# bacpop/ska.rust

Hardware: AMD Instinct MI355X
Metric: genomes/sec ska build+align, 1 000x5 Mbp k=31; bit-exact vs CPU (higher is better)
Workload: dtype u64

## Files before the change

ska.rust_amd/csrc/skx_device.hip:

```cpp
#include "skx_device.h"
#include <cstdlib>

namespace skx {

HashParams make_hash_params(int k)
{
    HashParams p;
    p.bits = 2 * (k - 1);
    p.hb = k - 1;
    p.hmask = p.hb >= 32 ? ~0u : ((1u << p.hb) - 1);
    p.c[0] = 0x9E3779B1u; p.c[1] = 0x85EBCA6Bu; p.c[2] = 0xC2B2AE35u; p.c[3] = 0x27D4EB2Fu;
    return p;
}

__device__ static inline uint32_t revcomp_arm(uint32_t x, int n)
{
    x = __builtin_bitreverse32(x);
    x = ((x >> 1) & 0x55555555u) | ((x & 0x55555555u) << 1);
    x ^= 0xAAAAAAAAu;
    return n ? x >> (32 - 2 * n) : 0;
}

__device__ static inline void pack16(const uint32_t w[4], uint32_t &code, uint32_t &bad, uint32_t &nl)
{
// ... 15 lines not shown
}
__device__ static inline void pack16_nonl(const uint32_t w[4], uint32_t &code, uint32_t &bad)
{
    code = 0; bad = 0;
    uint32_t c0f = 0x0F0F0F0Fu, c7f = 0x7F7F7F7Fu;
    asm volatile("" : "+v"(c0f), "+v"(c7f));
#pragma unroll
    for (int i = 0; i < 4; i++) {
        uint32_t x = w[i];
        uint32_t c = (x >> 1) & 0x03030303u;
        code = (code << 8) | ((c * 0x40100401u) >> 24);
        uint32_t t = (x & c0f) ^ 0x0E0E0E0Eu;
        uint32_t nzt = (t + c7f) & 0x80808080u;
        uint32_t u = x ^ 0x0A0A0A0Au;
        uint32_t znl = ~(((u & c7f) + c7f) | u | c7f);
        uint32_t fb = (((~nzt) & 0x80808080u) | znl) >> 7;
        bad |= (((fb * 0x01020408u) >> 24) & 0xFu) << (4 * i);
    }
}
__device__ static inline uint32_t qualbad16(const uint32_t w[4], int min_qual)
{
    uint32_t m = 0;
#pragma unroll
    for (int i = 0; i < 4; i++)
#pragma unroll
        for (int b = 0; b < 4; b++) {
            uint32_t q = (w[i] >> (8 * b)) & 0xFF;
            m |= (uint32_t)(((q - 33u) & 0xFFu) <= (uint32_t)min_qual) << (4 * i + b);
        }
    return m;
}

__device__ static inline uint32_t block_excl_scan(uint32_t v, uint32_t *s_tmp, uint32_t *total);
__device__ static inline uint32_t block_excl_scan_row(uint32_t v, uint32_t *s_tmp, uint32_t *total, int tid);

#ifdef SKX_PHASE_PROF
__device__ unsigned long long g_phase_prof[1024 * 16];
#define PHASE_PROF_(i) do { if (threadIdx.x == 0) { const unsigned long long t_ = __builtin_readcyclecounter(); atomicAdd(&g_phase_prof[(blockIdx.x & 1023) * 16 + (i)], t_ - tprof); tprof = t_; } } while (0)
#define PHASE_PROF_START unsigned long long tprof = __builtin_readcyclecounter()
extern "C" void skx_debug_phase_prof(unsigned long long *out, int reset)
{
    static unsigned long long h[1024 * 16];
    (void)hipDeviceSynchronize();
    (void)hipMemcpyFromSymbol(h, HIP_SYMBOL(g_phase_prof), sizeof(h));
    for (int i = 0; i < 16; i++) { out[i] = 0; for (int j = 0; j < 1024; j++) out[i] += h[j * 16 + i]; }
    if (reset) { for (auto &x : h) x = 0; (void)hipMemcpyToSymbol(HIP_SYMBOL(g_phase_prof), h, sizeof(h)); }
}
#else
#define PHASE_PROF_(i) do { } while (0)
#define PHASE_PROF_START do { } while (0)
#endif
#if defined(SKX_PHASE_PROF) && SKX_PHASE_PROF == 1
#define EXT_PROF(i) do { if (SCATTER) PHASE_PROF_(i); } while (0)
#else
#define EXT_PROF(i) do { } while (0)
#endif
#if defined(SKX_PHASE_PROF) && SKX_PHASE_PROF == 4
#define UN_PROF(i) do { if ((threadIdx.x & 63) == 0) { const unsigned long long t_ = __builtin_readcyclecounter(); atomicAdd(&g_phase_prof[(blockIdx.x & 1023) * 16 + (i)], t_ - tprof); tprof = t_; } } while (0)
#define UN_WAIT() asm volatile("s_waitcnt vmcnt(0)" ::: "memory")
#else
#define UN_PROF(i) do { } while (0)
#define UN_WAIT() do { } while (0)
#endif
#if defined(SKX_PHASE_PROF) && SKX_PHASE_PROF == 2
#define DD_PROF(i) PHASE_PROF_(i)
#else
#define DD_PROF(i) do { } while (0)
#endif
template <bool SCATTER, int TILE, bool HI, int PPT, bool SPLIT, int RMAX>
__global__ __launch_bounds__(TILE / PPT, SPLIT ? 6 : 1) void extract_kernel(ExtractArgs a)
{
    constexpr int NT = TILE / PPT;
    constexpr int NCH = PPT / 16;
    constexpr int NCHUNK = TILE / 16 + 5;
    extern __shared__ __attribute__((aligned(16))) unsigned char s_raw[];
    const int B = 1 << a.logB;
    uint32_t *s_hist = reinterpret_cast<uint32_t *>(s_raw);
    uint32_t *s_base = s_hist + B + 4;
    uint32_t *s_tmp = s_base + B;
    unsigned char *s_rest = reinterpret_cast<unsigned char *>(s_tmp + 20);
    uint32_t *s_code = reinterpret_cast<uint32_t *>(s_rest);
    uint16_t *s_bad = reinterpret_cast<uint16_t *>(s_code + NCHUNK + 3);
    uint16_t *s_qbad = s_bad + NCHUNK + 3;
    uint64_t *s_stage = reinterpret_cast<uint64_t *>(s_rest);

    const int tid = threadIdx.x;
    PHASE_PROF_START;
    const uint64_t per_group = 8ull * (uint64_t)a.tiles_max;
    const uint64_t L = blockIdx.x;
    int sample; uint64_t tile;
    if (a.parts > 1) {
        const int v = (int)(L & 7u);
        if (v >= a.n_samples * a.parts) return;
        sample = v / a.parts; tile = (uint64_t)(v % a.parts) * (uint64_t)a.tiles_part + (L >> 3);
        if (tile >= (uint64_t)a.tiles_max || (L >> 3) >= (uint64_t)a.tiles_part) return;
    } else { sample = (int)((L / per_group) * 8 + (L % per_group) % 8); tile = (L % per_group) / 8; }
    if (sample >= a.n_samples) return;
    const uint64_t len = a.lens[sample];
    const uint64_t T0 = tile * TILE;
    if (T0 >= len) return;
    typedef const uint8_t __attribute__((address_space(1))) *gbytes_t;
    typedef uint32_t u32x4 __attribute__((ext_vector_type(4)));
    typedef const u32x4 __attribute__((address_space(1))) *gvec_t;
    gbytes_t seq = (gbytes_t)(uintptr_t)a.seqs[sample];
    gbytes_t qual = a.quals ? (gbytes_t)(uintptr_t)a.quals[sample] : (gbytes_t)0;

    const int k = a.k, h = (k - 1) / 2;
    const HashParams hp = a.hp;
    const int hb = hp.hb;
    const int bshift = hp.bits - a.logB;
    const int bsh_hi = hp.bits + 4 - 32 - a.logB;
    const uint32_t rcflag = a.rc ? ~0u : 0u;
    const bool top_from_hl = a.logB <= hb;
    const int top_shift = top_from_hl ? hb - a.logB : 0;
    const uint32_t am = (1u << (2 * h)) - 1;

    for (int i = tid; i < B + 4; i += NT) s_hist[i] = 0;
    for (int c = tid; c < NCHUNK; c += NT) {
        const int64_t p = (int64_t)T0 - 64 + 16 * (int64_t)c;
        uint32_t w[4], q[4] = {0, 0, 0, 0};
        if (p >= 0 && (uint64_t)p + 16 <= len) {
            const u32x4 v = *(gvec_t)(seq + p);
            w[0] = v.x; w[1] = v.y; w[2] = v.z; w[3] = v.w;
            if (qual) { const u32x4 u = *(gvec_t)(qual + p); q[0] = u.x; q[1] = u.y; q[2] = u.z; q[3] = u.w; }
        } else {
#pragma unroll
            for (int i = 0; i < 4; i++) {
                uint32_t x = 0, y = 0;
#pragma unroll
                for (int b = 0; b < 4; b++) {
                    int64_t pos = p + 4 * i + b;
                    bool in = pos >= 0 && (uint64_t)pos < len;
                    x |= (uint32_t)(in ? seq[pos] : (uint8_t)'\n') << (8 * b);
                    if (qual) y |= (uint32_t)(in ? qual[pos] : (uint8_t)'~') << (8 * b);
                }
                w[i] = x; q[i] = y;
            }
        }
        uint32_t code, bad;
        pack16_nonl(w, code, bad);
        uint32_t qb = 0;
        if (qual) {
            uint32_t c2, b2, nl;
            pack16(w, c2, b2, nl);
            qb = qualbad16(q, a.min_qual) & ~nl;
            if (a.qual_filter == 2) bad |= qb;
        }
        s_code[c] = code; s_bad[c] = (uint16_t)bad; if (qual) s_qbad[c] = (uint16_t)qb;
    }
    __syncthreads();
    EXT_PROF(0);
    constexpr uint64_t PF_AHEAD = 20;
    uint32_t pfw = 0;
    if (SCATTER && tid < TILE / 128) {
        uint64_t pos = T0 + PF_AHEAD * TILE + (uint64_t)tid * 128;
        gbytes_t ps = seq;
        uint64_t plen = len;
        if (T0 + PF_AHEAD * TILE >= len && sample + 8 < a.n_samples) {
            pos = (tile + PF_AHEAD - (len + TILE - 1) / TILE) * TILE + (uint64_t)tid * 128;
            ps = (gbytes_t)(uintptr_t)a.seqs[sample + 8]; plen = a.lens[sample + 8];
        }
        if (pos + 4 <= plen) pfw = *(const uint32_t __attribute__((address_space(1))) *)(ps + pos);
    }

    uint64_t wv[PPT];
    uint32_t rk[PPT];
    {
    const int c0 = tid * NCH + 4;
    const uint64_t prev = ((uint64_t)s_code[c0 - 2] << 32) | s_code[c0 - 1];
    uint32_t lower = (uint32_t)prev & am;
    uint32_t mid = (uint32_t)(prev >> (2 * h)) & 3u;
    uint32_t upper = (uint32_t)(prev >> (2 * h + 2)) & am;
    uint32_t rc_upper = revcomp_arm(lower, h), rc_lower = revcomp_arm(upper, h), rc_mid = mid ^ 2u;
#pragma unroll
    for (int half = 0; half < NCH; half++) {
        const int c = c0 + half;
        const uint64_t G = ~((uint64_t)s_bad[c - 2] | ((uint64_t)s_bad[c - 1] << 16) | ((uint64_t)s_bad[c] << 32)) & 0xFFFFFFFFFFFFull;
        uint64_t Wk = ~0ull;
        {
            uint64_t A = G; int offset = 0, span = 1;
            for (int bit = 0; bit < 6; bit++) {
                if ((k >> bit) & 1) { Wk &= A << offset; offset += span; }
                A &= A << span; span <<= 1;
            }
        }
        uint64_t V = Wk;
        const uint64_t cand = Wk & ~(G << k) & ((~G >> 1) | ((uint64_t)(s_bad[c + 1] & 1u) << 47)) & (0xFFFFull << 32);
        if (cand) {
            const int64_t pc = (int64_t)T0 - 64 + 16 * (int64_t)c;
            uint32_t m = (uint32_t)(cand >> 32);
            while (m) {
                const int j = __builtin_ctz(m); m &= m - 1;
                const uint64_t pos = (uint64_t)(pc + j + 1);
                if (pos >= len || seq[pos] == (uint8_t)'\n') V &= ~(1ull << (32 + j));
            }
        }
        if (qual && a.qual_filter != 0)
            V &= ~((((uint64_t)s_qbad[c - 2] | ((uint64_t)s_qbad[c - 1] << 16) | ((uint64_t)s_qbad[c] << 32))) << h);
        const uint32_t vm = (uint32_t)(V >> 32) & 0xFFFFu;
        const uint32_t cw = s_code[c];
#pragma unroll
        for (int j = 0; j < 16; j++) {
            const uint32_t code = (cw >> (30 - 2 * j)) & 3u;
            upper = ((upper << 2) | mid) & am;
            mid = lower >> (2 * h - 2);
            lower = ((lower << 2) | code) & am;
            rc_lower = (rc_lower >> 2) | (rc_mid << (2 * h - 2));
            rc_mid = mid ^ 2u;
            rc_upper = (rc_upper >> 2) | ((code ^ 2u) << (2 * h - 2));
            const uint64_t kf = ((uint64_t)upper << 32) | lower, kr = ((uint64_t)rc_upper << 32) | rc_lower;
            const bool gt = kf > kr && rcflag;
            const bool eq = kf == kr && rcflag;
            uint32_t hl = gt ? rc_upper : upper, hr = gt ? rc_lower : lower;
            const uint32_t m4 = (1u << (gt ? rc_mid : mid)) | (eq ? (1u << rc_mid) : 0u);
            hmix_halves(hl, hr, hp);
            const uint64_t w = ((uint64_t)hl << (hb + 4)) | ((uint64_t)hr << 4) | m4;
            wv[16 * half + j] = w;
            const bool valid = (vm >> j) & 1u;
            const uint32_t bk = valid ? (top_from_hl ? hl >> top_shift : (uint32_t)((w >> 4) >> bshift)) : (uint32_t)B;
            const uint32_t r = atomicAdd(&s_hist[bk], 1u);
            rk[16 * half + j] = (bk << 16) | r;
        }
    }
    }
    __syncthreads();
    EXT_PROF(1);
    uint32_t *ghist = a.hist + ((uint64_t)sample << a.logB);
    if (!SCATTER) {
        for (int i = tid; i < B; i += NT) { uint32_t n = s_hist[i]; if (n) atomicAdd(&ghist[i], n); }
        return;
    }
    const int R = (B + NT - 1) / NT;
    const int b0 = tid * R < B ? tid * R : B, b1 = b0 + R < B ? b0 + R : B;
    uint32_t gb[RMAX], lsum = 0;
#pragma unroll
    for (int r = 0; r < RMAX; r++) {
        gb[r] = 0;
        if (b0 + r < b1) { const uint32_t n = s_hist[b0 + r]; if (n) gb[r] = atomicAdd(&ghist[b0 + r], n); lsum += n; }
    }
    uint32_t total;
    uint32_t lrun = block_excl_scan_row(lsum, s_tmp, &total, tid);
    EXT_PROF(2);
#pragma unroll
    for (int r = 0; r < RMAX; r++)
        if (b0 + r < b1) { const uint32_t n = s_hist[b0 + r]; s_hist[b0 + r] = lrun; lrun += n; }
    if (tid == 0) s_hist[B] = total;
    __syncthreads();
    EXT_PROF(3);
    constexpr uint32_t HALF = SPLIT ? TILE / 2 : TILE;
    uint32_t sidx_[SPLIT ? PPT : 1];
#pragma unroll
    for (int j = 0; j < PPT; j++) {
        const uint32_t idx = s_hist[rk[j] >> 16] + (rk[j] & 0xFFFFu);
        if (SPLIT) sidx_[j] = idx;
        if (idx < HALF) s_stage[idx] = wv[j];
    }
    const uint64_t *off = a.off + ((uint64_t)sample << a.logB);
    const bool fixed = a.capacity != 0xFFFFFFFFu;
    const uint64_t span0 = fixed ? ((uint64_t)sample << a.logB) * a.capacity : off[0];
    bool dropped = false;
#pragma unroll
    for (int r = 0; r < RMAX; r++)
        if (b0 + r < b1) {
            const uint32_t b = (uint32_t)(b0 + r), start = s_hist[b], n = s_hist[b + 1] - start;
            const bool over = n && gb[r] + n > a.capacity;
            if (over) dropped = true;
            s_base[b] = over ? 0u - start : (fixed ? b * a.capacity : (uint32_t)(off[b] - off[0])) + gb[r] - start;
        }
    asm volatile("" :: "v"(pfw));
    __syncthreads();
    EXT_PROF(4);
    typedef uint64_t __attribute__((address_space(1))) *gout_t;
    gout_t out = (gout_t)(uintptr_t)(a.words + span0);
    const uint32_t end0 = total < HALF ? total : HALF;
    for (uint32_t i = tid; i < end0; i += NT) {
        const uint64_t w = s_stage[i];
        const uint32_t b = HI ? (uint32_t)(w >> 32) >> bsh_hi : (uint32_t)((w >> 4) >> bshift);
        out[s_base[b] + i] = w;
    }
    EXT_PROF(5);
    if (SPLIT && total > HALF) {
        __syncthreads();
        EXT_PROF(6);
#pragma unroll
        for (int j = 0; j < PPT; j++) if (sidx_[j] - HALF < HALF) s_stage[sidx_[j] - HALF] = wv[j];
        __syncthreads();
        EXT_PROF(7);
        for (uint32_t i = HALF + tid; i < total; i += NT) {
            const uint64_t w = s_stage[i - HALF];
            const uint32_t b = HI ? (uint32_t)(w >> 32) >> bsh_hi : (uint32_t)((w >> 4) >> bshift);
            out[s_base[b] + i] = w;
        }
    }
    EXT_PROF(8);
    if (dropped) *a.overflow = 1;
}
template <int TILE, bool SPLIT>
static inline size_t extract_lds(const ExtractArgs &a, bool scatter)
{
    size_t codes = (size_t)(TILE / 16 + 8) * 8 + 64;
    size_t stage = scatter ? (size_t)TILE * (SPLIT ? 4 : 8) : 0;
    return ((size_t)8 << a.logB) + 16 + 80 + (stage > codes ? stage : codes);
}
static inline void extract_parts(ExtractArgs &a)
{
    a.parts = 0; a.tiles_part = 0;
    if (a.n_samples >= 1 && a.n_samples < 8 && a.tiles_max >= 64) { a.parts = 8 / a.n_samples; a.tiles_part = (a.tiles_max + a.parts - 1) / a.parts; if (a.parts < 2) a.parts = 0; }
}
template <bool SCATTER, int TILE, bool HI, int PPT, bool SPLIT, int RMAX>
static void launch_extract_t(const ExtractArgs &a_, hipStream_t st)
{
    ExtractArgs a = a_;
    extract_parts(a);
    const uint64_t g = a.parts > 1 ? 8ull * (uint64_t)a.tiles_part : (((uint64_t)a.n_samples + 7) / 8) * 8ull * (uint64_t)a.tiles_max;
    if (!g) return;
    const size_t lds = extract_lds<TILE, SPLIT>(a, SCATTER);
    (void)hipFuncSetAttribute((const void *)extract_kernel<SCATTER, TILE, HI, PPT, SPLIT, RMAX>, hipFuncAttributeMaxDynamicSharedMemorySize, (int)lds);
    hipLaunchKernelGGL((extract_kernel<SCATTER, TILE, HI, PPT, SPLIT, RMAX>), dim3((unsigned)g), dim3(TILE / PPT), lds, st, a);
}
template <bool SCATTER>
static void launch_extract(const ExtractArgs &a, hipStream_t st)
{
    const bool hi = a.hp.bits + 4 - 32 - a.logB >= 0;
    if (a.logB <= 10) {
        if (hi) launch_extract_t<SCATTER, 12288, true, 16, SCATTER, 2>(a, st); else launch_extract_t<SCATTER, 12288, false, 16, SCATTER, 2>(a, st);
    } else if (a.logB == 11) {
        if (hi) launch_extract_t<SCATTER, 12288, true, 16, SCATTER, 4>(a, st); else launch_extract_t<SCATTER, 12288, false, 16, SCATTER, 4>(a, st);
    } else {
        if (hi) launch_extract_t<SCATTER, 8192, true, 16, SCATTER, 16>(a, st); else launch_extract_t<SCATTER, 8192, false, 16, SCATTER, 16>(a, st);
    }
}
int extract_tile_bases(int logB) { return logB <= 11 ? 12288 : 8192; }
void launch_hist(const ExtractArgs &a, hipStream_t st) { launch_extract<false>(a, st); }
void launch_scatter(const ExtractArgs &a, hipStream_t st)
{
    launch_extract<true>(a, st);
}
__device__ static inline uint32_t wave_incl_scan(uint32_t v)
{
    const int lane = threadIdx.x & 63;
#pragma unroll
    for (int d = 1; d < 64; d <<= 1) { uint32_t t = __shfl_up(v, d, 64); if (lane >= d) v += t; }
    return v;
}
__device__ static inline uint32_t block_excl_scan(uint32_t v, uint32_t *s_tmp , uint32_t *total)
{
    const int lane = threadIdx.x & 63, wv = threadIdx.x >> 6, nw = (blockDim.x + 63) >> 6;
    uint32_t inc = wave_incl_scan(v);
    if (lane == 63) s_tmp[wv] = inc;
    __syncthreads();
    if (threadIdx.x == 0) { uint32_t run = 0; for (int i = 0; i < nw; i++) { uint32_t t = s_tmp[i]; s_tmp[i] = run; run += t; } s_tmp[16] = run; }
    __syncthreads();
    uint32_t r = s_tmp[wv] + inc - v;
    if (total) *total = s_tmp[16];
    __syncthreads();
    return r;
}

__device__ static inline uint32_t wave_incl_scan_dpp(uint32_t v)
{
    uint32_t inc = v;
    inc += (uint32_t)__builtin_amdgcn_update_dpp(0, (int)inc, 0x111, 0xf, 0xf, true);
    inc += (uint32_t)__builtin_amdgcn_update_dpp(0, (int)inc, 0x112, 0xf, 0xf, true);
    inc += (uint32_t)__builtin_amdgcn_update_dpp(0, (int)inc, 0x114, 0xf, 0xf, true);
    inc += (uint32_t)__builtin_amdgcn_update_dpp(0, (int)inc, 0x118, 0xf, 0xf, true);
    inc += (uint32_t)__builtin_amdgcn_update_dpp(0, (int)inc, 0x142, 0xa, 0xf, false);
    inc += (uint32_t)__builtin_amdgcn_update_dpp(0, (int)inc, 0x143, 0xc, 0xf, false);
    return inc;
}
__device__ static inline uint32_t block_excl_scan_row(uint32_t v, uint32_t *s_tmp , uint32_t *total, int tid)
{
    const int lane = tid & 63;
    const int wv = __builtin_amdgcn_readfirstlane(tid >> 6), nw = (int)((blockDim.x + 63) >> 6);
    const uint32_t inc = wave_incl_scan_dpp(v);
    if (lane == 63) s_tmp[wv] = inc;
    __syncthreads();
    uint32_t t = lane < nw ? s_tmp[lane & 15] : 0u;
    t += (uint32_t)__builtin_amdgcn_update_dpp(0, (int)t, 0x111, 0xf, 0xf, true);
    t += (uint32_t)__builtin_amdgcn_update_dpp(0, (int)t, 0x112, 0xf, 0xf, true);
    t += (uint32_t)__builtin_amdgcn_update_dpp(0, (int)t, 0x114, 0xf, 0xf, true);
    t += (uint32_t)__builtin_amdgcn_update_dpp(0, (int)t, 0x118, 0xf, 0xf, true);
    const uint32_t before = wv ? (uint32_t)__builtin_amdgcn_readlane((int)t, wv - 1) : 0u;
    if (total) *total = (uint32_t)__builtin_amdgcn_readlane((int)t, nw - 1);
    return before + inc - v;
}

__global__ __launch_bounds__(1024) void scan_u32_kernel(const uint32_t *in, uint64_t *out, uint64_t n, uint32_t *max_out)
{
    __shared__ uint32_t s_tmp[17];
    __shared__ uint32_t s_max;
    uint64_t carry = 0;
    uint32_t mx = 0;
    if (threadIdx.x == 0) s_max = 0;
    for (uint64_t base = 0; base < n; base += 4096) {
        uint32_t v[4]; uint32_t sum = 0;
#pragma unroll
        for (int i = 0; i < 4; i++) { uint64_t idx = base + (uint64_t)threadIdx.x * 4 + i; v[i] = idx < n ? in[idx] : 0; sum += v[i]; mx = v[i] > mx ? v[i] : mx; }
        uint32_t tot;
        uint32_t ex = block_excl_scan(sum, s_tmp, &tot);
        uint64_t run = carry + ex;
#pragma unroll
        for (int i = 0; i < 4; i++) { uint64_t idx = base + (uint64_t)threadIdx.x * 4 + i; if (idx < n) out[idx] = run; run += v[i]; }
        carry += tot;
    }
    if (threadIdx.x == 0) out[n] = carry;
    if (max_out) { atomicMax(&s_max, mx); __syncthreads(); if (threadIdx.x == 0) *max_out = s_max; }
}
__global__ void fill_offsets_kernel(uint64_t *off, uint64_t n, uint32_t capacity)
{
    for (uint64_t i = blockIdx.x * (uint64_t)blockDim.x + threadIdx.x; i <= n; i += (uint64_t)gridDim.x * blockDim.x) off[i] = i * capacity;
}
void launch_fill_offsets(uint64_t *off, uint64_t n, uint32_t capacity, hipStream_t st)
{
    hipLaunchKernelGGL(fill_offsets_kernel, dim3(1024), dim3(256), 0, st, off, n, capacity);
}
void launch_scan_u32(const uint32_t *in, uint64_t *out, uint64_t n, uint32_t *max_out, hipStream_t st)
{
    hipLaunchKernelGGL(scan_u32_kernel, dim3(1), dim3(1024), 0, st, in, out, n, max_out);
}

constexpr int SCAN8_PER_BLOCK = 8192;
__global__ __launch_bounds__(1024) void scan_u8_sums_kernel(const uint8_t *in, uint64_t n, uint32_t *sums)
{
    __shared__ uint32_t s_tmp[17];
    const uint64_t base = (uint64_t)blockIdx.x * SCAN8_PER_BLOCK + (uint64_t)threadIdx.x * 8;
    uint32_t sum = 0;
    if (base + 8 <= n) { uint64_t v = *reinterpret_cast<const uint64_t *>(in + base); for (int i = 0; i < 8; i++) sum += ((v >> (8 * i)) & 0xFF) == 1; }
    else for (int i = 0; i < 8; i++) sum += (base + i < n) && in[base + i] == 1;
    uint32_t tot; block_excl_scan(sum, s_tmp, &tot);
    if (threadIdx.x == 0) sums[blockIdx.x] = tot;
}
__global__ __launch_bounds__(1024) void scan_u8_apply_kernel(const uint8_t *in, uint64_t n, const uint64_t *block_off, uint64_t *out)
{
    __shared__ uint32_t s_tmp[17];
    const uint64_t base = (uint64_t)blockIdx.x * SCAN8_PER_BLOCK + (uint64_t)threadIdx.x * 8;
    uint32_t v[8]; uint32_t sum = 0;
    for (int i = 0; i < 8; i++) { v[i] = (base + i < n) && in[base + i] == 1; sum += v[i]; }
    uint32_t ex = block_excl_scan(sum, s_tmp, nullptr);
    uint64_t run = block_off[blockIdx.x] + ex;
    for (int i = 0; i < 8; i++) { if (base + i < n) out[base + i] = run; run += v[i]; }
    if (blockIdx.x == gridDim.x - 1 && threadIdx.x == blockDim.x - 1) out[n] = run;
}
uint64_t scan_u8_blocks(uint64_t n) { return (n + SCAN8_PER_BLOCK - 1) / SCAN8_PER_BLOCK; }
void launch_scan_u8(const uint8_t *flags, uint64_t *pos, uint64_t n, uint32_t *sums, uint64_t *offs, hipStream_t st)
{
    const uint64_t nb = scan_u8_blocks(n);
    if (nb == 0) { (void)hipMemsetAsync(pos, 0, 8, st); return; }
    hipLaunchKernelGGL(scan_u8_sums_kernel, dim3((unsigned)nb), dim3(1024), 0, st, flags, n, sums);
    hipLaunchKernelGGL(scan_u32_kernel, dim3(1), dim3(1024), 0, st, (const uint32_t *)sums, offs, nb, (uint32_t *)nullptr);
    hipLaunchKernelGGL(scan_u8_apply_kernel, dim3((unsigned)nb), dim3(1024), 0, st, flags, n, (const uint64_t *)offs, pos);
}

constexpr uint32_t TABLE_PAD = 128;

template <bool HI>
__device__ static inline uint32_t word_field(uint64_t w, int sh, uint32_t mask)
{
    return HI ? ((uint32_t)(w >> 32) >> (sh - 32)) & mask : (uint32_t)(w >> sh) & mask;
}

__device__ static inline uint32_t home_slot(uint64_t w, int rem_bits, uint32_t nslots)
{
    uint32_t l32;
    if (rem_bits >= 32) {
        const int sh = rem_bits - 28;
        l32 = sh >= 32 ? (uint32_t)(w >> 32) : __builtin_amdgcn_alignbit((uint32_t)(w >> 32), (uint32_t)w, (uint32_t)sh);
    } else {
        l32 = rem_bits == 0 ? 0u : (uint32_t)(((w >> 4) & ((1ull << rem_bits) - 1)) << (32 - rem_bits));
    }
    return __umulhi(l32, nslots);
}
template <bool FAST>
__device__ static inline uint32_t home_slot_t(uint64_t w, int rem_bits, uint32_t nslots)
{
    if (FAST) return __umulhi(__builtin_amdgcn_alignbit((uint32_t)(w >> 32), (uint32_t)w, (uint32_t)(rem_bits - 28)), nslots);
    return home_slot(w, rem_bits, nslots);
}
__device__ static inline bool table_insert(unsigned long long *tab, uint32_t total_slots, uint32_t home, uint64_t w)
{
    const uint64_t key = w >> 4;
    for (uint32_t i = home; i < total_slots; ++i) {
        unsigned long long old = tab[i];
        if (old == 0ull) old = atomicCAS(&tab[i], 0ull, (unsigned long long)w);
        if (old == 0ull) return true;
        if ((old >> 4) == key) {
            if ((old | w) != old) atomicOr(&tab[i], (unsigned long long)(w & 15ull));
            return true;
        }
    }
    return false;
}
__device__ static inline int table_insert_slot(unsigned long long *tab, uint32_t total_slots, uint32_t home, uint64_t w, uint32_t &slot)
{
    const uint64_t key = w >> 4;
    for (uint32_t i = home; i < total_slots; ++i) {
        unsigned long long old = tab[i];
        bool mine = false;
        if (old == 0ull) { old = atomicCAS(&tab[i], 0ull, (unsigned long long)w); mine = old == 0ull; }
        if (mine) { slot = i; return 2; }
        if ((old >> 4) == key) {
            if ((old | w) != old) atomicOr(&tab[i], (unsigned long long)(w & 15ull));
            slot = i; return 1;
        }
    }
    return 0;
}
template <typename F>
__device__ static inline uint32_t table_emit_sorted(const unsigned long long *tab, uint32_t total_slots, uint32_t *s_tmp, F f)
{
    const uint32_t per = (total_slots + blockDim.x - 1) / blockDim.x;
    const uint32_t lo = threadIdx.x * per;
    const uint32_t hi = lo + per < total_slots ? lo + per : total_slots;
    uint32_t cnt = 0;
    for (uint32_t i = lo; i < hi; i++) cnt += tab[i] != 0ull;
    uint32_t total;
    uint32_t c = block_excl_scan(cnt, s_tmp, &total);
    for (uint32_t i = lo; i < hi; i++) {
        const unsigned long long w = tab[i];
        if (!w) continue;
        uint32_t gl = 0, lr = 0;
        for (int64_t j = (int64_t)i - 1; j >= 0; j--) { unsigned long long o = tab[j]; if (!o) break; gl += o > w; }
        for (uint32_t j = i + 1; j < total_slots; j++) { unsigned long long o = tab[j]; if (!o) break; lr += o < w; }
        f(c - gl + lr, (uint64_t)w);
        c++;
    }
    return total;
}
template <typename F>
__device__ static inline uint32_t table_emit_sorted_slot(const unsigned long long *tab, uint32_t total_slots, uint32_t *s_tmp, F f)
{
    const uint32_t per = (total_slots + blockDim.x - 1) / blockDim.x;
    const uint32_t lo = threadIdx.x * per;
    const uint32_t hi = lo + per < total_slots ? lo + per : total_slots;
    uint32_t cnt = 0;
    for (uint32_t i = lo; i < hi; i++) cnt += tab[i] != 0ull;
    uint32_t total;
    uint32_t c = block_excl_scan(cnt, s_tmp, &total);
    for (uint32_t i = lo; i < hi; i++) {
        const unsigned long long w = tab[i];
        if (!w) continue;
        uint32_t gl = 0, lr = 0;
        for (int64_t j = (int64_t)i - 1; j >= 0; j--) { unsigned long long o = tab[j]; if (!o) break; gl += o > w; }
        for (uint32_t j = i + 1; j < total_slots; j++) { unsigned long long o = tab[j]; if (!o) break; lr += o < w; }
        f(c - gl + lr, (uint64_t)w, i);
        c++;
    }
    return total;
}

typedef const uint64_t __attribute__((address_space(1))) *gwords_t;
__device__ static inline gwords_t as_global(const uint64_t *p) { return (gwords_t)(uintptr_t)p; }

__global__ __launch_bounds__(256) void dedupe_kernel(uint64_t *words, const uint64_t *off, const uint32_t *raw, uint32_t *ucnt,
                                                     uint32_t nslots, int rem_bits, int *overflow, uint32_t min_n, uint16_t *sidx, int sb)
{
    extern __shared__ __attribute__((aligned(16))) unsigned long long s_tab[];
    __shared__ uint32_t s_tmp[17];
    __shared__ uint32_t s_sub[SUBIDX];
    __shared__ int s_fail;
    const uint64_t region = blockIdx.x;
    const uint32_t n = raw[region];
    if (n <= min_n) return;
    if (n == 0) { if (threadIdx.x == 0) ucnt[region] = 0; if (threadIdx.x < SUBIDX) sidx[region * SUBIDX + threadIdx.x] = 0; return; }
    if (threadIdx.x < SUBIDX) s_sub[threadIdx.x] = 0xFFFFFFFFu;
    const uint32_t total_slots = nslots + TABLE_PAD;
    for (uint32_t i = threadIdx.x; i < total_slots; i += blockDim.x) s_tab[i] = 0ull;
    if (threadIdx.x == 0) s_fail = 0;
    __syncthreads();
    uint64_t *reg = words + off[region];
    for (uint32_t i = threadIdx.x; i < n; i += blockDim.x) {
        const uint64_t w = reg[i];
        if (!table_insert(s_tab, total_slots, home_slot(w, rem_bits, nslots), w)) s_fail = 1;
    }
    __syncthreads();
    if (s_fail) { if (threadIdx.x == 0) { *overflow = 1; ucnt[region] = 0; } if (threadIdx.x < SUBIDX) sidx[region * SUBIDX + threadIdx.x] = 0; return; }
    const uint64_t lmask = rem_bits >= 60 ? ~0ull : ((1ull << rem_bits) - 1);
    uint32_t total = table_emit_sorted(s_tab, total_slots, s_tmp, [&](uint32_t idx, uint64_t w) {
        reg[idx] = w;
        atomicMin(&s_sub[sb ? (uint32_t)(((w >> 4) & lmask) >> (rem_bits - sb)) : 0u], idx);
    });
    if (threadIdx.x == 0) ucnt[region] = total;
    __syncthreads();
    if (threadIdx.x < SUBIDX) {
        uint32_t v = total;
        for (int s2 = SUBIDX - 1; s2 >= (int)threadIdx.x; s2--) if (s_sub[s2] != 0xFFFFFFFFu) v = s_sub[s2];
        sidx[region * SUBIDX + threadIdx.x] = (uint16_t)v;
    }
}
void launch_dedupe(uint64_t *words, const uint64_t *off, const uint32_t *raw, uint32_t *ucnt, uint64_t n_regions,
                   uint32_t table_slots, int rem_bits, int *overflow, uint32_t min_n, uint16_t *sidx, int sb, hipStream_t st)
{
    if (!n_regions) return;
    size_t lds = (size_t)(table_slots + TABLE_PAD) * 8;
    (void)hipFuncSetAttribute((const void *)dedupe_kernel, hipFuncAttributeMaxDynamicSharedMemorySize, (int)lds);
    hipLaunchKernelGGL(dedupe_kernel, dim3((unsigned)n_regions), dim3(256), lds, st, words, off, raw, ucnt, table_slots, rem_bits, overflow, min_n, sidx, sb);
}

template <int ITEMS, bool HI, int NT>
__global__ __launch_bounds__(NT) void dedupe_mb_kernel(uint64_t *words, const uint64_t *off, const uint32_t *raw, uint32_t *ucnt,
                                                        uint32_t cap, int rem_bits, int *overflow, uint16_t *sidx, int sb,
                                                        const uint32_t *big, uint32_t big_from, int big_mode)
{
    extern __shared__ __attribute__((aligned(16))) unsigned char s_mem[];
    __shared__ uint32_t s_tmp[17];
    PHASE_PROF_START;
    uint64_t region = blockIdx.x;
    if (big_mode == 2) {
        const uint32_t cnt = big[0], idx = big_from + blockIdx.x;
        if (blockIdx.x == 0 && threadIdx.x == 0 && cnt > big_from + gridDim.x) atomicOr(overflow, 4);
        if (idx >= cnt) return;
        region = big[1 + idx];
    }
    const uint32_t n = raw[region];
    if (n == 0) { if (threadIdx.x == 0) ucnt[region] = 0; return; }
    if (big_mode == 1 && n > (uint32_t)NT * ITEMS) return;
    if (n > cap || n > (uint32_t)NT * ITEMS) { if (threadIdx.x == 0) atomicOr(overflow, 2); return; }
    uint64_t *s_elem = reinterpret_cast<uint64_t *>(s_mem);
    uint32_t *s_cnt = reinterpret_cast<uint32_t *>(s_mem + (size_t)cap * 8 + 32) + 1;
    int logM = 31 - __clz(n);
    if (logM < 0) logM = 0;
    if (logM > rem_bits) logM = rem_bits;
    while ((1u << logM) > cap) logM--;
    const uint32_t M = 1u << logM;
    const int mshift = rem_bits - logM + 4;
    uint64_t *reg = words + off[region];
    uint64_t e[ITEMS];
#pragma unroll
    for (int t = 0; t < ITEMS; t++) { const uint32_t i = threadIdx.x + (uint32_t)NT * t; e[t] = i < n ? reg[i] : 0ull; }
    for (uint32_t i = threadIdx.x; i < M; i += NT) s_cnt[i] = 0;
    if (threadIdx.x == 0) s_cnt[-1] = 0;
    if (threadIdx.x < 4) s_elem[n + threadIdx.x] = ~0ull;
    __syncthreads();
    DD_PROF(0);
#pragma unroll
    for (int t = 0; t < ITEMS; t++) if (e[t]) atomicAdd(&s_cnt[word_field<HI>(e[t], mshift, M - 1)], 1u);
// ... 772 lines not shown
```

Measured before the change: 29120.

## Add persistent warp-specialized scatter kernel with async double-buffered text loads

```diff
diff --git a/ska.rust_amd/csrc/skx_device.hip b/ska.rust_amd/csrc/skx_device.hip
--- a/ska.rust_amd/csrc/skx_device.hip
+++ b/ska.rust_amd/csrc/skx_device.hip
@@ -341,6 +341,258 @@
     size_t stage = scatter ? (size_t)TILE * (SPLIT ? 4 : 8) : 0;
     return ((size_t)8 << a.logB) + 16 + 80 + (stage > codes ? stage : codes);
 }
+
+__device__ static inline uint32_t wave_incl_scan_dpp(uint32_t v);
+template <bool SCATTER, int TILE, bool HI, int PPT, int LOGB>
+__global__ __launch_bounds__(TILE / PPT + 64, 4) void extract_kernel(ExtractArgs a)
+{
+    constexpr int NT = TILE / PPT;
+    constexpr int NCW = NT / 64;
+    constexpr int NCH = PPT / 16;
+    constexpr int NCHUNK = TILE / 16 + 5;
+    constexpr int TEXT = NCHUNK * 16;
+    constexpr int NDMA = (NCHUNK + 63) / 64;
+    constexpr int B = 1 << LOGB;
+    constexpr int R = (B + NT - 1) / NT;
+    constexpr int NBL = B / 64;
+    constexpr uint32_t ROUND = 8192, NROUND = (TILE + ROUND - 1) / ROUND;
+    static_assert(SCATTER && PPT % 16 == 0 && NCW <= 16 && B % 64 == 0 && TILE < 65536 && (NCHUNK + 3) * 6 <= (int)ROUND * 8, "");
+    extern __shared__ __attribute__((aligned(16))) unsigned char s_raw[];
+    uint32_t *s_hist = reinterpret_cast<uint32_t *>(s_raw);
+    uint32_t *s_base = s_hist + B + 4;
+    uint32_t *s_tmp = s_base + B;
+    unsigned char *s_text = reinterpret_cast<unsigned char *>(s_tmp + 16);
+    unsigned char *s_rest = s_text + 2 * TEXT;
+    uint32_t *s_code = reinterpret_cast<uint32_t *>(s_rest);
+    uint16_t *s_bad = reinterpret_cast<uint16_t *>(s_code + NCHUNK + 3);
+    uint64_t *s_stage = reinterpret_cast<uint64_t *>(s_rest);
+    auto bar = []() { asm volatile("s_waitcnt lgkmcnt(0)\n\ts_barrier" ::: "memory"); };
+
+    const int tid = threadIdx.x, lane = tid & 63;
+    typedef const uint8_t __attribute__((address_space(1))) *gbytes_t;
+    typedef uint32_t u32x4 __attribute__((ext_vector_type(4)));
+    const int xcd = (int)(blockIdx.x & 7u), slot = (int)(blockIdx.x >> 3), nslot = (int)(gridDim.x >> 3);
+    const bool parts = a.parts > 1;
+    if (parts && xcd >= a.n_samples * a.parts) return;
+    const int64_t n_items = parts ? (int64_t)a.tiles_part : (int64_t)((a.n_samples + 7) / 8) * a.tiles_max;
+    auto item_at = [&](int64_t i, int &sample, uint64_t &tile) {
+        if (parts) { sample = xcd / a.parts; tile = (uint64_t)(xcd % a.parts) * (uint64_t)a.tiles_part + (uint64_t)i; }
+        else { sample = (int)(i / a.tiles_max) * 8 + xcd; tile = (uint64_t)(i % a.tiles_max); }
+    };
+    auto next_item = [&](int64_t i) -> int64_t {
+        for (; i < n_items; i += nslot) {
+            int s; uint64_t t; item_at(i, s, t);
+            if (s < a.n_samples && t < (uint64_t)a.tiles_max && t * TILE < a.lens[s]) return i;
+        }
+        return n_items;
+    };
+    const bool fixed = a.capacity != 0xFFFFFFFFu;
+    int64_t item = next_item(slot);
+    if (item >= n_items) return;
+
+    if (__builtin_amdgcn_readfirstlane(tid >> 6) == NCW) {
+        auto load_text = [&](int64_t i, int buf) {
+            int s; uint64_t t; item_at(i, s, t);
+            const uint64_t len = a.lens[s];
+            gbytes_t seq = (gbytes_t)(uintptr_t)a.seqs[s];
+#pragma unroll
+            for (int u = 0; u < NDMA; u++) {
+                const int c = 64 * u + lane;
+                const int64_t p = (int64_t)(t * TILE) - 64 + 16 * (int64_t)c;
+                if (c < NCHUNK && p >= 0 && (uint64_t)p + 16 <= len)
+                    __builtin_amdgcn_global_load_lds((__attribute__((address_space(1))) void *)(uintptr_t)(seq + p),
+                                                     (__attribute__((address_space(3))) void *)(s_text + buf * TEXT + 1024 * u), 16, 0, 0);
+            }
+        };
+        bool dropped = false;
+        load_text(item, 0);
+        asm volatile("s_waitcnt vmcnt(0)" ::: "memory");
+        bar();
+        for (int it = 0; item < n_items; it++) {
+            const int64_t nxt = next_item(item + nslot);
+            int sample; uint64_t tile; item_at(item, sample, tile);
+            bar(); bar();
+            uint32_t *ghist = a.hist + ((uint64_t)sample << LOGB);
+            uint32_t gb[NBL];
+#pragma unroll
+            for (int u = 0; u < NBL; u++) { const uint32_t n = s_hist[64 * u + lane]; gb[u] = n ? atomicAdd(&ghist[64 * u + lane], n) : 0u; }
+            bar(); bar();
+            const uint64_t *off = a.off + ((uint64_t)sample << LOGB);
+#pragma unroll
+            for (int u = 0; u < NBL; u++) s_base[64 * u + lane] = gb[u];
+#pragma unroll 1
+            for (int u = 0; u < NBL; u++) {
+                const uint32_t b = (uint32_t)(64 * u + lane), start = s_hist[b], n = s_hist[b + 1] - start, g0 = s_base[b];
+                const bool over = n && g0 + n > a.capacity;
+                if (over) dropped = true;
+                s_base[b] = over ? 0u - start : (fixed ? b * a.capacity : (uint32_t)(off[b] - off[0])) + g0 - start;
+            }
+            if (nxt < n_items) load_text(nxt, (it & 1) ^ 1);
+            for (uint32_t rd = 0; rd < NROUND; rd++) {
+                bar();
+                if (rd + 1 == NROUND) asm volatile("s_waitcnt vmcnt(0)" ::: "memory");
+                bar();
+            }
+            item = nxt;
+        }
+        if (dropped) *a.overflow = 1;
+        return;
+    }
+
+    const int k = a.k, h = (k - 1) / 2;
+    const HashParams hp = a.hp;
+    const int hb = hp.hb;
+    const int bshift = hp.bits - LOGB;
+    const int bsh_hi = hp.bits + 4 - 32 - LOGB;
+    const uint32_t rcflag = a.rc ? ~0u : 0u;
+    const bool top_from_hl = LOGB <= hb;
+    const int top_shift = top_from_hl ? hb - LOGB : 0;
+    const uint32_t am = (1u << (2 * h)) - 1;
+    const int b0 = tid * R < B ? tid * R : B, b1 = b0 + R < B ? b0 + R : B;
+    bar();
+    for (int it = 0; item < n_items; it++) {
+        const int64_t nxt = next_item(item + nslot);
+        int sample; uint64_t tile; item_at(item, sample, tile);
+        const uint64_t len = a.lens[sample];
+        const uint64_t T0 = tile * TILE;
+        gbytes_t seq = (gbytes_t)(uintptr_t)a.seqs[sample];
+        unsigned char *text = s_text + (it & 1) * TEXT;
+
+        for (int i = tid; i < B + 4; i += NT) s_hist[i] = 0;
+        for (int c = tid; c < NCHUNK; c += NT) {
+            const int64_t p = (int64_t)T0 - 64 + 16 * (int64_t)c;
+            uint32_t w[4];
+            if (p >= 0 && (uint64_t)p + 16 <= len) {
+                const u32x4 v = *reinterpret_cast<const u32x4 *>(text + 16 * c);
+                w[0] = v.x; w[1] = v.y; w[2] = v.z; w[3] = v.w;
+            } else {
+#pragma unroll
+                for (int i = 0; i < 4; i++) {
+                    uint32_t x = 0;
+#pragma unroll
+                    for (int b = 0; b < 4; b++) {
+                        const int64_t pos = p + 4 * i + b;
+                        x |= (uint32_t)(pos >= 0 && (uint64_t)pos < len ? seq[pos] : (uint8_t)'\n') << (8 * b);
+                    }
+                    w[i] = x;
+                }
+                u32x4 v; v.x = w[0]; v.y = w[1]; v.z = w[2]; v.w = w[3];
+                *reinterpret_cast<u32x4 *>(text + 16 * c) = v;
+            }
+            uint32_t code, bad;
+            pack16_nonl(w, code, bad);
+            s_code[c] = code; s_bad[c] = (uint16_t)bad;
+        }
+        bar();
+        uint64_t wv[PPT];
+        uint32_t rk[PPT];
+        {
+            const int c0 = tid * NCH + 4;
+            const uint64_t prev = ((uint64_t)s_code[c0 - 2] << 32) | s_code[c0 - 1];
+            uint32_t lower = (uint32_t)prev & am;
+            uint32_t mid = (uint32_t)(prev >> (2 * h)) & 3u;
+            uint32_t upper = (uint32_t)(prev >> (2 * h + 2)) & am;
+            uint32_t rc_upper = revcomp_arm(lower, h), rc_lower = revcomp_arm(upper, h), rc_mid = mid ^ 2u;
+#pragma unroll
+            for (int half = 0; half < NCH; half++) {
+                const int c = c0 + half;
+                const uint64_t G = ~((uint64_t)s_bad[c - 2] | ((uint64_t)s_bad[c - 1] << 16) | ((uint64_t)s_bad[c] << 32)) & 0xFFFFFFFFFFFFull;
+                uint64_t Wk = ~0ull;
+                {
+                    uint64_t A = G; int offset = 0, span = 1;
+                    for (int bit = 0; bit < 6; bit++) {
+                        if ((k >> bit) & 1) { Wk &= A << offset; offset += span; }
+                        A &= A << span; span <<= 1;
+                    }
+                }
+                uint64_t V = Wk;
+                const uint64_t cand = Wk & ~(G << k) & ((~G >> 1) | ((uint64_t)(s_bad[c + 1] & 1u) << 47)) & (0xFFFFull << 32);
+                if (cand) {
+                    const int64_t pc = (int64_t)T0 - 64 + 16 * (int64_t)c;
+                    uint32_t m = (uint32_t)(cand >> 32);
+                    while (m) {
+                        const int j = __builtin_ctz(m); m &= m - 1;
+                        const uint64_t pos = (uint64_t)(pc + j + 1);
+                        if (pos >= len || text[pos - (T0 - 64)] == (uint8_t)'\n') V &= ~(1ull << (32 + j));
+                    }
+                }
+                const uint32_t vm = (uint32_t)(V >> 32) & 0xFFFFu;
+                const uint32_t cw = s_code[c];
+#pragma unroll
+                for (int j = 0; j < 16; j++) {
+                    const uint32_t code = (cw >> (30 - 2 * j)) & 3u;
+                    upper = ((upper << 2) | mid) & am;
+                    mid = lower >> (2 * h - 2);
+                    lower = ((lower << 2) | code) & am;
+                    rc_lower = (rc_lower >> 2) | (rc_mid << (2 * h - 2));
+                    rc_mid = mid ^ 2u;
+                    rc_upper = (rc_upper >> 2) | ((code ^ 2u) << (2 * h - 2));
+                    const uint64_t kf = ((uint64_t)upper << 32) | lower, kr = ((uint64_t)rc_upper << 32) | rc_lower;
+                    const bool gt = kf > kr && rcflag;
+                    const bool eq = kf == kr && rcflag;
+                    uint32_t hl = gt ? rc_upper : upper, hr = gt ? rc_lower : lower;
+                    const uint32_t m4 = (1u << (gt ? rc_mid : mid)) | (eq ? (1u << rc_mid) : 0u);
+                    hmix_halves(hl, hr, hp);
+                    const uint64_t w = ((uint64_t)hl << (hb + 4)) | ((uint64_t)hr << 4) | m4;
+                    wv[16 * half + j] = w;
+                    const bool valid = (vm >> j) & 1u;
+                    const uint32_t bk = valid ? (top_from_hl ? hl >> top_shift : (uint32_t)((w >> 4) >> bshift)) : (uint32_t)B;
+                    const uint32_t r = atomicAdd(&s_hist[bk], 1u);
+                    rk[16 * half + j] = (bk << 16) | r;
+                }
+            }
+        }
+        bar();
+        uint32_t lsum = 0;
+#pragma unroll
+        for (int r = 0; r < R; r++) if (b0 + r < b1) lsum += s_hist[b0 + r];
+        const uint32_t inc = wave_incl_scan_dpp(lsum);
+        if (lane == 63) s_tmp[tid >> 6] = inc;
+        bar();
+        uint32_t total;
+        {
+            const int wvi = __builtin_amdgcn_readfirstlane(tid >> 6);
+            uint32_t t = lane < NCW ? s_tmp[lane & 15] : 0u;
+            t += (uint32_t)__builtin_amdgcn_update_dpp(0, (int)t, 0x111, 0xf, 0xf, true);
+            t += (uint32_t)__builtin_amdgcn_update_dpp(0, (int)t, 0x112, 0xf, 0xf, true);
+            t += (uint32_t)__builtin_amdgcn_update_dpp(0, (int)t, 0x114, 0xf, 0xf, true);
+            t += (uint32_t)__builtin_amdgcn_update_dpp(0, (int)t, 0x118, 0xf, 0xf, true);
+            uint32_t lrun = (wvi ? (uint32_t)__builtin_amdgcn_readlane((int)t, wvi - 1) : 0u) + inc - lsum;
+            total = (uint32_t)__builtin_amdgcn_readlane((int)t, NCW - 1);
+#pragma unroll
+            for (int r = 0; r < R; r++)
+                if (b0 + r < b1) { const uint32_t n = s_hist[b0 + r]; s_hist[b0 + r] = lrun; lrun += n; }
+            if (tid == 0) s_hist[B] = total;
+        }
+        bar();
+#pragma unroll
+        for (int j = 0; j < PPT; j++) {
+            const uint32_t idx = s_hist[rk[j] >> 16] + (rk[j] & 0xFFFFu);
+            rk[j] = idx;
+            if (idx < ROUND) s_stage[idx] = wv[j];
+            if ((j & 7) == 7) asm volatile("" ::: "memory");
+        }
+        const uint64_t span0 = fixed ? ((uint64_t)sample << LOGB) * a.capacity : a.off[(uint64_t)sample << LOGB];
+        typedef uint64_t __attribute__((address_space(1))) *gout_t;
+        gout_t out = (gout_t)(uintptr_t)(a.words + span0);
+#pragma unroll
+        for (uint32_t rd = 0; rd < NROUND; rd++) {
+            if (rd > 0) {
+#pragma unroll
+                for (int j = 0; j < PPT; j++) if (rk[j] - rd * ROUND < ROUND) s_stage[rk[j] - rd * ROUND] = wv[j];
+            }
+            bar();
+            const uint32_t end = total < (rd + 1) * ROUND ? total : (rd + 1) * ROUND;
+            for (uint32_t i = rd * ROUND + tid; i < end; i += NT) {
+                const uint64_t w = s_stage[i - rd * ROUND];
+                const uint32_t b = HI ? (uint32_t)(w >> 32) >> bsh_hi : (uint32_t)((w >> 4) >> bshift);
+                out[s_base[b] + i] = w;
+            }
+            bar();
+        }
+        item = nxt;
+    }
+}
 static inline void extract_parts(ExtractArgs &a)
 {
     a.parts = 0; a.tiles_part = 0;
@@ -357,6 +609,19 @@
     (void)hipFuncSetAttribute((const void *)extract_kernel<SCATTER, TILE, HI, PPT, SPLIT, RMAX>, hipFuncAttributeMaxDynamicSharedMemorySize, (int)lds);
     hipLaunchKernelGGL((extract_kernel<SCATTER, TILE, HI, PPT, SPLIT, RMAX>), dim3((unsigned)g), dim3(TILE / PPT), lds, st, a);
 }
+template <bool HI>
+static void launch_extract_persistent(const ExtractArgs &a_, hipStream_t st)
+{
+    constexpr int TILE = 24576, PPT = 32, LOGB = 11, NCHUNK = TILE / 16 + 5;
+    ExtractArgs a = a_;
+    extract_parts(a);
+    int dev = 0, cus = 0;
+    if (hipGetDevice(&dev) != hipSuccess || hipDeviceGetAttribute(&cus, hipDeviceAttributeMultiprocessorCount, dev) != hipSuccess) cus = 0;
+    const unsigned g = (unsigned)(cus >= 16 ? cus / 8 * 8 : 8);
+    const size_t lds = (size_t)4 * ((1 << LOGB) + 4) + (size_t)4 * (1 << LOGB) + 64 + (size_t)2 * 16 * NCHUNK + (size_t)8 * 8192;
+    (void)hipFuncSetAttribute((const void *)extract_kernel<true, TILE, HI, PPT, LOGB>, hipFuncAttributeMaxDynamicSharedMemorySize, (int)lds);
+    hipLaunchKernelGGL((extract_kernel<true, TILE, HI, PPT, LOGB>), dim3(g), dim3(TILE / PPT + 64), lds, st, a);
+}
 template <bool SCATTER>
 static void launch_extract(const ExtractArgs &a, hipStream_t st)
 {
@@ -364,12 +629,18 @@
     if (a.logB <= 10) {
         if (hi) launch_extract_t<SCATTER, 12288, true, 16, SCATTER, 2>(a, st); else launch_extract_t<SCATTER, 12288, false, 16, SCATTER, 2>(a, st);
     } else if (a.logB == 11) {
-        if (hi) launch_extract_t<SCATTER, 12288, true, 16, SCATTER, 4>(a, st); else launch_extract_t<SCATTER, 12288, false, 16, SCATTER, 4>(a, st);
+        if (SCATTER && !a.quals) {
+            if (hi) launch_extract_persistent<true>(a, st); else launch_extract_persistent<false>(a, st);
+            return;
+        }
+        ExtractArgs b = a;
+        b.tiles_max = 2 * a.tiles_max;
+        if (hi) launch_extract_t<SCATTER, 12288, true, 16, SCATTER, 4>(b, st); else launch_extract_t<SCATTER, 12288, false, 16, SCATTER, 4>(b, st);
     } else {
         if (hi) launch_extract_t<SCATTER, 8192, true, 16, SCATTER, 16>(a, st); else launch_extract_t<SCATTER, 8192, false, 16, SCATTER, 16>(a, st);
     }
 }
-int extract_tile_bases(int logB) { return logB <= 11 ? 12288 : 8192; }
+int extract_tile_bases(int logB) { return logB <= 10 ? 12288 : logB == 11 ? 24576 : 8192; }
 void launch_hist(const ExtractArgs &a, hipStream_t st) { launch_extract<false>(a, st); }
 void launch_scatter(const ExtractArgs &a, hipStream_t st)
 {
```

New measurement: 29130 (median of 5 runs). Within noise of the previous version (+0.0%).
